# Hfx-J/SGTD

Measured on AMD Instinct MI355X. Metric: query frames/sec vs map size (descriptor build + candidate selection), higher is better.
Workload: dtype f64

## Files before the change

### sgtd_amd/csrc/order_kernels.hip.h

```cpp
#pragma once
#include "probe_kernels.hip.h"

#define SGTD_OS_THREADS 512
#define SGTD_OS_ITEMS 16
#define SGTD_OS_TILE (SGTD_OS_THREADS * SGTD_OS_ITEMS)
#define SGTD_GI_THREADS 256
#define SGTD_GI_ITEMS 16
#define SGTD_GI_TILE (SGTD_GI_THREADS * SGTD_GI_ITEMS)
#define SGTD_ORDER_WINDOW 8
#define SGTD_ORDER_POLLS_DEFAULT (1u << 20)
#define SGTD_ORDER_MAX_KEYS (1ll << 30)

enum { OW_TICKET = 0, OW_GROUP_TICKET = 4, OW_HIST = 64, OW_STATE = OW_HIST + 4 * 256 };
__host__ __device__ __forceinline__ size_t order_sort_state_at(int pass, u32 tiles_cap) { return (size_t)OW_STATE + (size_t)pass * tiles_cap * 256; }
__host__ __device__ __forceinline__ size_t order_group_state_at(int passes, u32 tiles_cap) { return (order_sort_state_at(passes, tiles_cap) + 1) & ~(size_t)1; }
__host__ __device__ __forceinline__ size_t order_work_words(int passes, u32 tiles_cap, u32 gtiles_cap) { return order_group_state_at(passes, tiles_cap) + (size_t)gtiles_cap * 2; }

#define SGTD_ST_AGG 1u
#define SGTD_ST_INCL 2u
#define SGTD_ST_MASK 0x3FFFFFFFu

__device__ __forceinline__ u32 order_ld(const u32 *p) { return __hip_atomic_load(p, __ATOMIC_RELAXED, __HIP_MEMORY_SCOPE_AGENT); }
__device__ __forceinline__ void order_st(u32 *p, u32 v) { __hip_atomic_store(p, v, __ATOMIC_RELAXED, __HIP_MEMORY_SCOPE_AGENT); }
__device__ __forceinline__ u64 order_ld64(const u64 *p) { return __hip_atomic_load(p, __ATOMIC_RELAXED, __HIP_MEMORY_SCOPE_AGENT); }
__device__ __forceinline__ void order_st64(u64 *p, u64 v) { __hip_atomic_store(p, v, __ATOMIC_RELAXED, __HIP_MEMORY_SCOPE_AGENT); }

__global__ __launch_bounds__(256) void order_begin_kernel(const u32 *count, u32 *q_prefix, int n_queries, u32 *n_valid, u32 *q_M, unsigned long long *q_P) {
  __shared__ u32 lds[256 / SGTD_WAVE + 1];
  for (int q = threadIdx.x; q < n_queries; q += 256) { q_M[q] = 0u; q_P[q] = 0ull; }
  u32 carry = 0;
  for (int q0 = 0; q0 < n_queries; q0 += 256) {
    const int q = q0 + threadIdx.x;
    const u32 v = (q < n_queries) ? count[q] : 0;
    u32 tot;
    const u32 ex = block_excl_scan(v, lds, tot);
    if (q < n_queries) q_prefix[q] = carry + ex;
    carry += tot;
  }
  if (threadIdx.x == 0) *n_valid = carry;
}

__global__ __launch_bounds__(256) void home_keys_hist_kernel(QueryView Q, const u32 *q_prefix, u32 *keys, u32 *vals, long long n_slots, int cbits, int sub_bits,
                                                             u32 *hist, u32 *pos_of_slot, size_t n_pass_slots) {
  __shared__ u32 h[4 * 256];
  for (int i = threadIdx.x; i < 4 * 256; i += 256) h[i] = 0u;
  __syncthreads();
  const u64 cmask = (1ull << cbits) - 1ull;
  const int ny = 1 << (sub_bits >> 1), nz = 1 << (sub_bits - (sub_bits >> 1));
  for (long long d = (long long)blockIdx.x * 256 + threadIdx.x; d < n_slots; d += (long long)gridDim.x * 256) {
    const int q = (int)(d / Q.stride);
    const u32 i = (u32)(d - (long long)q * Q.stride);
    if (i >= Q.count[q]) continue;
    const u64 code = label_code(Q.label[d * 3 + 0], Q.label[d * 3 + 1], Q.label[d * 3 + 2]);
    const double s0 = Q.side[d * 3 + 0], s1 = Q.side[d * 3 + 1], s2 = Q.side[d * 3 + 2];
    const u64 x = home_coord(s0, cmask), y = home_coord(s1, cmask), z = home_coord(s2, cmask);
    const double f1 = s1 - (double)(int)s1, f2 = s2 - (double)(int)s2;
    const u64 sub = (u64)min(max((int)(f1 * ny), 0), ny - 1) * nz + (u64)min(max((int)(f2 * nz), 0), nz - 1);
    const u32 key = (u32)(((((code << cbits | x) << cbits | y) << cbits) | z) << sub_bits | sub);
    const u32 idx = q_prefix[q] + i;
    keys[idx] = key;
    vals[idx] = (u32)d;
#pragma unroll
    for (int b = 0; b < 4; b++) atomicAdd(&h[b * 256 + ((key >> (8 * b)) & 255u)], 1u);
  }
  __syncthreads();
  for (int i = threadIdx.x; i < 4 * 256; i += 256)
    if (h[i]) atomicAdd(&hist[i], h[i]);
  uint4 *p4 = reinterpret_cast<uint4 *>(pos_of_slot);
  const size_t n4 = n_pass_slots / 4, step = (size_t)gridDim.x * 256, first = (size_t)blockIdx.x * 256 + threadIdx.x;
  for (size_t i = first; i < n4; i += step) p4[i] = make_uint4(SGTD_NO_PASS, SGTD_NO_PASS, SGTD_NO_PASS, SGTD_NO_PASS);
  for (size_t i = n4 * 4 + first; i < n_pass_slots; i += step) pos_of_slot[i] = SGTD_NO_PASS;
}

__global__ __launch_bounds__(SGTD_OS_THREADS) __attribute__((amdgpu_waves_per_eu(4))) void order_sort_pass_kernel(
const u32 *keys_in, const u32 *vals_in, u32 *keys_out, u32 *vals_out,
                                                                          const u32 *n_valid_p, long long n_cap, u32 *work, u32 tiles_cap, int pass,
                                                                          u32 max_polls, u32 *giveup) {
  constexpr int NW = SGTD_OS_THREADS / SGTD_WAVE;
  constexpr u32 PER_WAVE = SGTD_OS_TILE / NW;
  __shared__ u32 s_key[SGTD_OS_TILE], s_val[SGTD_OS_TILE];
  __shared__ u32 s_wcnt[NW][256];
  __shared__ u32 s_start[256];
  __shared__ u32 s_gbase[256];
  __shared__ u32 s_scan[NW + 1];
  __shared__ u32 s_tile, s_quit;
  const u32 tid = threadIdx.x, wid = tid >> 6, lane = tid & 63u;
  const u32 nv = (u32)min((long long)*n_valid_p, n_cap);
  const u32 ntiles = min((nv + SGTD_OS_TILE - 1u) / SGTD_OS_TILE, tiles_cap);
  if (blockIdx.x >= ntiles) return;
  if (tid == 0) { s_tile = atomicAdd(&work[OW_TICKET + pass], 1u); s_quit = order_ld(giveup); }
  for (u32 i = tid; i < NW * 256u; i += SGTD_OS_THREADS) (&s_wcnt[0][0])[i] = 0u;
  __syncthreads();
  const u32 tile = s_tile;
  if (s_quit || tile >= ntiles) return;
// ... 189 lines not shown
    s_heads = c_heads; s_last = c_last;
  }
  __syncthreads();
  if (s_quit) return;
  u32 H = s_heads + ex_heads, F = ex_last ? ex_last : s_last;
  u32 g[SGTD_GI_ITEMS];
#pragma unroll
  for (int j = 0; j < SGTD_GI_ITEMS; j++) {
    const u32 p = p0 + j;
    if ((heads >> j) & 1u) { H++; F = p + 1u; }
    g[j] = H - 1u;
    if (p < nv) {
      if (((heads >> j) & 1u) && H <= nv) group_first[H - 1u] = p;
      if (!pair) pos_of_slot[p] = p;
      else {
        const u32 f = F - 1u;
        if (((p - f) % SGTD_PAIR) == 0u) {
          const u32 s = (H - 1u) + (f + SGTD_PAIR - 1u) / SGTD_PAIR + (p - f) / SGTD_PAIR;
          if (s < slot_cap) pos_of_slot[s] = p;
        }
      }
      if (p == nv - 1u) *n_groups = H;
    }
  }
  if (full) {
    uint4 *dst = reinterpret_cast<uint4 *>(gid + p0);
#pragma unroll
    for (int j = 0; j < SGTD_GI_ITEMS / 4; j++) dst[j] = make_uint4(g[4 * j], g[4 * j + 1], g[4 * j + 2], g[4 * j + 3]);
  } else {
#pragma unroll
    for (int j = 0; j < SGTD_GI_ITEMS; j++) if (p0 + j < nv) gid[p0 + j] = g[j];
  }
}
```

### sgtd_amd/csrc/probe_kernels.hip.h

```cpp
#pragma once
#include "common.hip.h"
#include <type_traits>

struct TableView {
  const HotEntry *ent;
  IdMap map;
  const double *cold_side;
  const BucketDir *dir;
  const HashSlot *hash;
  u32 hash_mask;
  u32 n_entries;
  u32 frame_lo;
  u32 frame_span;
  u32 coarse_at;
  u32 whole_at;
  u32 tail_off;
  const BucketDir *dir1;
  const HashSlot *hash1;
  u32 hash_mask1;
  u32 n_entries1;
};
__host__ __device__ __forceinline__ u32 group_row_bytes(const TableView &T) { return T.tail_off ? 2u * SGTD_GROUP_ROW_BYTES : SGTD_GROUP_ROW_BYTES; }

struct QueryView {
// ... 64 lines not shown
struct WaveSlab {
  u32 state;
  u64 swept;
#ifdef SGTD_EXP_PHASE
  u64 ph[8], t;
#endif
};
#ifdef SGTD_EXP_PHASE
__device__ unsigned long long g_phase[8];
#define PH_ADD(i) do { const u64 _n = __builtin_readcyclecounter(); slab.ph[i] += _n - slab.t; slab.t = _n; } while (0)
#else
#define PH_ADD(i) do { } while (0)
#endif

__global__ __launch_bounds__(256) void query_prefix_kernel(const u32 *count, u32 *q_prefix, int n_queries,
                                                           u32 *n_valid) {
  __shared__ u32 lds[256 / SGTD_WAVE + 1];
  u32 carry = 0;
  for (int q0 = 0; q0 < n_queries; q0 += 256) {
    const int q = q0 + threadIdx.x;
    const u32 v = (q < n_queries) ? count[q] : 0;
    u32 tot;
    const u32 ex = block_excl_scan(v, lds, tot);
    if (q < n_queries) q_prefix[q] = carry + ex;
    carry += tot;
  }
  if (threadIdx.x == 0) *n_valid = carry;
}

__device__ __forceinline__ u64 home_coord(double s, u64 cmask) {
  return (int)(s - 1.0) < 0 ? cmask : min((u64)(u32)(int)s, cmask);
}

template <class KeyT>
__global__ void home_keys_kernel(QueryView Q, const u32 *q_prefix, KeyT *keys, u32 *vals, long long n_slots,
                                 int cbits, int sub_bits) {
  const long long d = (long long)blockIdx.x * blockDim.x + threadIdx.x;
  if (d >= n_slots) return;
  const int q = (int)(d / Q.stride);
  const u32 i = (u32)(d - (long long)q * Q.stride);
  if (i >= Q.count[q]) return;
  const u64 code = label_code(Q.label[d * 3 + 0], Q.label[d * 3 + 1], Q.label[d * 3 + 2]);
  const u64 cmask = (1ull << cbits) - 1ull;
  const u64 x = home_coord(Q.side[d * 3 + 0], cmask), y = home_coord(Q.side[d * 3 + 1], cmask),
            z = home_coord(Q.side[d * 3 + 2], cmask);
  const u32 idx = q_prefix[q] + i;
  const int ny = 1 << (sub_bits >> 1), nz = 1 << (sub_bits - (sub_bits >> 1));
  const double f1 = Q.side[d * 3 + 1] - (double)(int)Q.side[d * 3 + 1], f2 = Q.side[d * 3 + 2] - (double)(int)Q.side[d * 3 + 2];
  const u64 sub = (u64)min(max((int)(f1 * ny), 0), ny - 1) * nz + (u64)min(max((int)(f2 * nz), 0), nz - 1);
  keys[idx] = (KeyT)(((((code << cbits | x) << cbits | y) << cbits) | z) << sub_bits | sub);
  vals[idx] = (u32)d;
}

template <class KeyT>
__global__ void group_heads_kernel(const KeyT *keys, const u32 *n_valid_p, u32 *flags, long long n, int cbits, int sub_bits) {
  const long long p = (long long)blockIdx.x * blockDim.x + threadIdx.x;
  if (p >= n) return;
  u32 head = 0;
  if (p + 1 < (long long)*n_valid_p) {
    const u64 a = (u64)keys[p + 1] >> sub_bits, b = (u64)keys[p] >> sub_bits;
    const u64 cmask = (1ull << cbits) - 1ull;
    head = (a != b) || ((a & cmask) == cmask) || (((a >> cbits) & cmask) == cmask) ||
           (((a >> (2 * cbits)) & cmask) == cmask);
  }
  flags[p] = head;
}

__global__ void group_first_kernel(const u32 *gid, const u32 *n_valid_p, u32 *group_first, u32 *n_groups, long long n) {
  const long long p = (long long)blockIdx.x * blockDim.x + threadIdx.x;
  const long long nv = (long long)*n_valid_p;
  if (p >= n || p >= nv) return;
  const u32 g = gid[p];
  if (p == 0 || gid[p - 1] != g) group_first[g] = (u32)p;
  if (p == nv - 1) *n_groups = g + 1;
}

__global__ __launch_bounds__(256) void group_resolve_kernel(TableView T, QueryView Q, const u32 *order,
                                                            const u32 *group_first, const u32 *n_groups_p,
                                                            const u32 *n_valid_p, unsigned char *rows, u32 rows_cap,
                                                            int *overflow) {
  const int c = (int)(threadIdx.x & 31);
  const long long stride = ((long long)gridDim.x * blockDim.x) >> 5;
  const long long n_groups = (*n_valid_p) ? (long long)*n_groups_p : 0;
  if (n_groups > (long long)rows_cap) {
// ... 180 lines not shown
      head = (a != b) || ((a & cmask) == cmask) || (((a >> S.cbits) & cmask) == cmask) || (((a >> (2 * S.cbits)) & cmask) == cmask);
    }
    fl[j] = head;
    mine += head;
  }
  u32 tot;
  u32 ex = block_excl_scan(mine, s_sum, tot);
#pragma unroll
  for (u32 j = 0; j < PER; j++) {
    const u32 p = tid * PER + j;
    s_gid[p] = ex;
    if (p < S.n_slots) { S.gid[p] = ex; if (p < nv) S.order[p] = (u32)(s_key[p] & 8191ull); }
    ex += fl[j];
  }
  __syncthreads();
  for (u32 p = tid; p < nv; p += SGTD_SMALL_THREADS) {
    const u32 g = s_gid[p];
    if (p == 0 || s_gid[p - 1] != g) { s_first[g] = p; S.group_first[g] = p; }
  }
  if (tid == 0) { *S.n_valid = nv; *S.n_groups = nv ? s_gid[nv - 1] + 1u : 0u; }
  __syncthreads();
  for (u32 p = tid; p < nv; p += SGTD_SMALL_THREADS) {
    if (!S.pair) { S.pos_of_slot[p] = p; continue; }
    const u32 g = s_gid[p], f = s_first[g];
    if (((p - f) % SGTD_PAIR) == 0u) S.pos_of_slot[g + (f + SGTD_PAIR - 1u) / SGTD_PAIR + (p - f) / SGTD_PAIR] = p;
  }
}

__device__ __forceinline__ void reached_slices(float dq, float t_up, int n, int &lo, int &hi) {
  const float a = ((dq - t_up) + 0.5f) * (float)n - 1e-4f;
  const float b = ((dq + t_up) + 0.5f) * (float)n + 1e-4f;
  lo = !(a > 0.0f) ? 0 : (a >= (float)n ? n : (int)a);
  hi = b < 0.0f ? -1 : (!(b < (float)n) ? n - 1 : (int)b);
}

#ifndef SGTD_PLAN_GROUPS
#define SGTD_PLAN_GROUPS 16
#endif
#define SGTD_PLAN_THREADS 256
#ifndef SGTD_PLAN_WAVES
#define SGTD_PLAN_WAVES __attribute__((amdgpu_waves_per_eu(5)))
#endif
#ifndef SGTD_PLAN_INFLIGHT
#define SGTD_PLAN_INFLIGHT 4u
#endif
#ifndef SGTD_PLAN_SPARSE
#define SGTD_PLAN_SPARSE 1
#endif
#ifndef SGTD_PLAN_QUADS
#define SGTD_PLAN_QUADS 448
#endif
#define SGTD_ROW_QUADS (2 * SGTD_NCELL + 1)
template <bool PAIR, bool TAIL>
__global__ __launch_bounds__(SGTD_PLAN_THREADS) SGTD_PLAN_WAVES void plan_passes_kernel(TableView T, QueryView Q, const u32 *order, const u32 *gid,
                                                          const u32 *pos_of_slot, const u32 *n_valid_p,
                                                          const u32 *n_groups_p, const unsigned char *rows, u32 rows_cap, PassPool P,
                                                          u32 *n_visit, uint2 *list, int *overflow) {
  constexpr u32 SEGS = TAIL ? 2u : 1u;
  constexpr u32 NG = SGTD_PLAN_GROUPS / SEGS;
  constexpr size_t ROWB = (size_t)SEGS * SGTD_GROUP_ROW_BYTES;
  __shared__ uint4 s_rows[SGTD_PLAN_THREADS / SGTD_WAVE][SGTD_PLAN_QUADS + 2];
  const int lane = lane_id();
  uint4 *my_rows = s_rows[threadIdx.x >> 6];
  if (lane < 2) my_rows[lane] = make_uint4(0u, 0u, 0u, 0u);
  __builtin_amdgcn_wave_barrier();
  const u32 nv = *n_valid_p;
// ... 1400 lines not shown
```

### sgtd_amd/csrc/sgtd_accel.hip

```cpp
#include "../../include/sgtd_accel.h"

#include <hip/hip_runtime.h>

#include <algorithm>
#include <atomic>
#include <chrono>
#include <cmath>
#include <cstdio>
#include <cstring>
#include <limits>
#include <memory>
#include <string>
#include <vector>

#include "build_kernel.hip.h"
#include "common.hip.h"
#include "table_kernels.hip.h"
#include "probe_kernels.hip.h"
#include "order_kernels.hip.h"
#include "select_kernels.hip.h"
#include "verify_kernels.hip.h"
#include "verify_mfma.hip.h"
#include "exchange_kernels.hip.h"
#include "remove_kernels.hip.h"
// ... 60 lines not shown
  T *p = nullptr;
  size_t n = 0, cap = 0;
  PinnedVec() = default;
  PinnedVec(const PinnedVec &) = delete;
  PinnedVec &operator=(const PinnedVec &) = delete;
  ~PinnedVec() { if (p) (void)hipHostFree(p); }
  bool resize(size_t want) {
    if (want > cap) {
      void *np = nullptr;
      const size_t c = std::max<size_t>(want + want / 4, 64);
      if (hipHostMalloc(&np, c * sizeof(T), hipHostMallocDefault) != hipSuccess) return false;
      if (p) (void)hipHostFree(p);
      p = static_cast<T *>(np);
      cap = c;
    }
    n = want;
    return true;
  }
  T *data() { return p; }
  const T *data() const { return p; }
  T &operator[](size_t i) { return p[i]; }
  const T &operator[](size_t i) const { return p[i]; }
  size_t size() const { return n; }
};

constexpr size_t kCtrWords = CTR_XCD_HEADS + 8 * 1024;
enum { EV_START = 0, EV_BUILD, EV_SORT, EV_PROBE, EV_VOTES, EV_TOPK, EV_COUNT_T, EV_SCAN, EV_WRITE, EV_COUNT };

struct SelectPlan {
  int nq = 0, cn = 0; long long n_slots = 0; u32 span = 1, frame_lo = 0, id_bits = 13;
  u32 chunk = SGTD_PROBE_CHUNK; int blocks = 0, groups = 0, agrid = 0;
  u32 tile_span = 1, n_tiles = 1; size_t hist_bytes = 0; bool lds_votes = false;
  bool votes_fit = false, table_fits = false, per_query = false, fused_pairs = false, fused_votes = false, votes_per_query = false;
  int cbits = 1, sub_bits = 0, key_bits = 0; bool small = false, pair = false; size_t max_pass_slots = 0;
  bool order_fused = false; u32 order_tiles = 0, order_gtiles = 0;
  int row_slots = 1; u32 ticket = 2; int sgrid = 0, pgrid = 0; bool narrow = false, frames = false;
  bool narrow_pairs = false;
};

}

namespace multi { struct Group; }

struct sgtd_engine {
  multi::Group *grp = nullptr;
  sgtd_config cfg;
  DevCfg dc;
  hipStream_t stream = nullptr;
  std::string err;
  int n_cus = 256;
  bool timing = false;
  hipEvent_t ev[EV_COUNT] = {};

  sgtd_engine *attached_to = nullptr;
  unsigned long long table_version = 0;
  unsigned long long attached_version = 0;
  int n_views = 0;
  u32 current_frame_id = 0;
  DescStore tab;
  int64_t n_entries = 0;
  int64_t n_add_calls = 0;
  bool have_frames = false;
  u32 frame_lo = 0, frame_hi = 0;
  bool finalized = false;

  struct Segment {
// ... 128 lines not shown
  std::vector<int64_t> sk_off, sk_kp_off;
  enum { LM_POSE = 0, LM_OFF, LM_ANCH, LM_COUNT, LM_MERGED, LM_MEM_OFF, LM_MEMBER, LM_SEG, LM_CNT, LM_START, LM_MPTS, LM_MLAB, LM_XYZ, LM_LABEL,
         LM_NPOINTS, LM_BUFS };
  DevBuf lm[LM_BUFS];
  int lm_n = -1, lm_passes = 0;
  int64_t lm_kept = 0;
  std::vector<int64_t> lm_kp_off, lm_mem_off, lm_merged;
  hipEvent_t lm_ev[3] = {nullptr, nullptr, nullptr};
  float lm_ms[3] = {0.f, 0.f, 0.f};
  int *export_packed = nullptr;
  size_t export_cap = 0;
  hipEvent_t ev_cand = nullptr, ev_export_free = nullptr;
  bool export_busy = false;
  u32 batch_serial = 0;
  bool defer_lists = false;
  bool lists_pending = false;
  bool lists_masked = false;
  const u64 *verify_keep = nullptr;
  const u64 *list_keep = nullptr;
  SelectPlan plan;
  DevBuf rough_qi, rough_entry, rough_frame, rough_cell, rough_dis;
  size_t rec_cap = (size_t)1 << 25;
  bool rec_cap_fixed = false;
  size_t pair_cap = (size_t)1 << 24;
  DevBuf n_valid, cell_rows, gid, q_prefix, group_first, n_groups;
  DevBuf pos_of_slot, rec_off, pass_pool;
  size_t pool_units = 0;
  size_t group_cap = 0;
  size_t group_cap_hook = 0;
  size_t amb_min = 65536;
  int sorted_chunk = 0;
  bool diag = false;
  int order_form = -1;
  u32 order_polls = SGTD_ORDER_POLLS_DEFAULT;
  bool order_gave_up = false;
  bool order_train = false;
  int select_mode = 0;
  PinnedVec<u32> h_count, h_pair_base, h_q_M;
  PinnedVec<unsigned long long> h_q_P;
  PinnedVec<int> h_n_cand, h_cand_frame, h_cand_votes;
  PinnedVec<long long> h_pair_off;
  sgtd_stats stats{};
  char *pin = nullptr;
  size_t pin_cap = 0, pin_used = 0;
  struct PinCopy { void *dst; size_t off, bytes; };
  std::vector<PinCopy> pin_pending;
};

#include "multi.hip.h"

namespace {

#define HIPCHK(call)                                                          \
  do {                                                                        \
    hipError_t _s = (call);                                                   \
    if (_s != hipSuccess) {                                                   \
      e->err = std::string(#call) + ": " + hipGetErrorString(_s);             \
      return SGTD_ERR_HIP;                                                    \
    }                                                                         \
  } while (0)
#define CHK(call)                 \
  do {                            \
    int _r = (call);              \
    if (_r != SGTD_OK) return _r; \
  } while (0)

// ... 574 lines not shown
  SelectPlan p;
  const int nq = p.nq = e->nq, cn = p.cn = e->dc.cand_num;
  const long long n_slots = p.n_slots = (long long)nq * e->q_stride;
  const u32 span = p.span = e->have_frames ? (e->frame_hi - e->frame_lo + 1) : 1;
  p.frame_lo = e->have_frames ? e->frame_lo : 0;
  p.id_bits = e->id_bits ? e->id_bits : 13;
  while (p.chunk > SGTD_SUB_DESCS && (long long)nq * ((e->q_stride + p.chunk - 1) / p.chunk) < 1024) p.chunk >>= 1;
  if (const char *o = getenv("SGTD_BLOCK_CHUNK")) { const int c = atoi(o); if (c == 32 || c == 64 || c == 128) p.chunk = (u32)c; }
  p.blocks = (int)((e->q_stride + p.chunk - 1) / p.chunk);
  p.groups = (p.blocks + 3) / 4;
  p.agrid = ((nq + 7) / 8) * p.groups * 8;
  p.tile_span = span <= 36 * 1024 ? span : 36 * 1024;
  p.n_tiles = (span + p.tile_span - 1) / p.tile_span;
  p.hist_bytes = (size_t)span * sizeof(u32);
  p.lds_votes = p.hist_bytes <= 150 * 1024;
  static const size_t votes_room = lds_room(&votes_topk_kernel), list_room = lds_room(&pairs_query_kernel<true>);
  p.votes_fit = votes_topk_lds_bytes(span) <= votes_room;
  p.table_fits = (size_t)SGTD_PQ_TILE_RECS * sizeof(u32) + (((size_t)span + 15) & ~(size_t)15) + 16 <= list_room;
  p.per_query = e->select_mode == 2 || (e->select_mode == 0 && nq >= e->n_cus && (p.votes_fit || p.table_fits));
  p.fused_pairs = p.per_query && !e->wide_pairs && p.id_bits <= SGTD_PQ_RANK_BITS && !(cn == SGTD_MAX_CAND && p.id_bits == SGTD_PQ_RANK_BITS);
  p.fused_votes = p.fused_pairs && p.votes_fit;
  p.votes_per_query = p.n_tiles == 1 ? nq >= e->n_cus : ((long long)nq * p.n_tiles >= e->n_cus / 4 && p.n_tiles <= 8);
  p.narrow_pairs = p.id_bits <= SGTD_NARROW_RANK_BITS && !e->wide_pairs;
  while ((1ll << p.cbits) < (long long)(e->dc.max_len * e->dc.scale) + 3 && p.cbits < 16) p.cbits++;
  const int spare = (8 - (12 + 3 * p.cbits) % 8) % 8;
  p.sub_bits = spare >= 2 ? std::min(spare, 6) : 4;
  if (const char *o = getenv("SGTD_HOME_SUB_BITS")) p.sub_bits = std::min(6, std::max(0, atoi(o)));
  p.key_bits = 12 + 3 * p.cbits + p.sub_bits;
  const bool small_on = [] { const char *o = getenv("SGTD_SMALL_ORDER"); return !(o && !atoi(o)); }();
  p.small = small_on && nq == 1 && n_slots <= SGTD_SMALL_SLOTS && p.key_bits <= 32 && !p.fused_votes && span <= (1u << 20);
  const bool small_shape = nq == 1 && n_slots <= SGTD_SMALL_SLOTS;
  p.order_fused = !p.small && (e->order_form == 1 || (e->order_form < 0 && !small_shape)) && !e->order_train && p.key_bits <= 32 && n_slots > 0 &&
                  n_slots < SGTD_ORDER_MAX_KEYS;
  p.order_tiles = (u32)((n_slots + SGTD_OS_TILE - 1) / SGTD_OS_TILE);
  p.order_gtiles = (u32)((n_slots + SGTD_GI_TILE - 1) / SGTD_GI_TILE);
  p.pair = !e->diag && SGTD_PAIR >= 2;
  p.max_pass_slots = (size_t)pass_slot_count((u32)n_slots, (u32)n_slots, p.pair) + 64;
  p.row_slots = e->n_seg > 1 ? 2 : 1;
  if (e->stats.last_D > 0 && e->stats.last_P_swept > 0) {
    const double per_pass = (double)e->stats.last_P_swept / ((double)e->stats.last_D / (p.pair ? kDescsPerPass : 1.0));
    p.ticket = (u32)std::min(8.0, std::max(1.0, std::floor(1536.0 / per_pass + 0.5)));
  }
  if (e->sorted_chunk > 0) p.ticket = (u32)std::min(SGTD_TICKET_MAX, e->sorted_chunk);
  p.sgrid = e->n_cus * 8;
  if (const char *o = getenv("SGTD_SWEEP_BLOCKS_PER_CU")) p.sgrid = e->n_cus * std::max(1, atoi(o));
  int plan_per_cu = 20;
  if (const char *o = getenv("SGTD_PLAN_BLOCKS_PER_CU")) plan_per_cu = std::max(1, atoi(o));
  p.pgrid = (int)std::min<long long>(grid_for((long long)p.max_pass_slots, SGTD_PLAN_THREADS), (long long)e->n_cus * plan_per_cu);
  const u32 n0 = (u32)(e->seg[0].g1 - e->seg[0].g0), n1 = (u32)(e->seg[1].g1 - e->seg[1].g0);
  p.narrow = ((unsigned long long)n0 + SGTD_SENTINELS + (e->n_seg > 1 ? n1 + SGTD_SENTINELS : 0u)) * sizeof(HotEntry) < (1ull << 32);
  p.frames = e->last_kind != 1 || (e->have_frames && e->last_qframe >= e->frame_lo && e->last_qframe <= e->frame_hi);
  return p;
}

Views make_views(sgtd_engine *e) {
  const SelectPlan &p = e->plan;
  Views v;
  v.span = p.span;
  TableView &T = v.T;
  const sgtd_engine::Segment &S = e->seg[0], &S1 = e->seg[1];
  T.ent = S.hot.as<HotEntry>(); T.map = id_map(e, p.id_bits); T.cold_side = e->tab.side.as<double>();
  T.dir = S.dir.as<BucketDir>();
  T.hash = S.hash.as<HashSlot>(); T.hash_mask = S.hash_mask;
  T.coarse_at = e->coarse_at; T.whole_at = e->whole_at;
  T.n_entries = (u32)(S.g1 - S.g0); T.frame_lo = p.frame_lo; T.frame_span = v.span;
  T.tail_off = e->n_seg > 1 ? T.n_entries + SGTD_SENTINELS : 0u;
// ... 237 lines not shown
}

int clear_batch(sgtd_engine *e, const SelectPlan &p) {
  const int nq = p.nq, cn = p.cn;
  if (e->thr2_pending > 0) {
    thr2_kernel<<<grid_for(e->thr2_pending, 256), 256, 0, e->stream>>>(e->qd.side.as<double>(), e->qd.frame.as<u32>(), e->qd.qrec.as<QueryRec>(), e->thr2_pending,
                                                                        e->dc.rough);
    HIPCHK(hipGetLastError());
  }
  if (p.small) return SGTD_OK;
  HIPCHK(hipMemsetAsync(e->cursors.p, 0, kCtrWords * sizeof(u32), e->stream));
  if (!p.fused_votes) {
    if (!p.votes_per_query) HIPCHK(hipMemsetAsync(e->votes.p, 0, (size_t)nq * p.span * sizeof(u32), e->stream));
    HIPCHK(hipMemsetAsync(e->slot_of.p, 0xFF, (size_t)nq * p.span, e->stream));
    HIPCHK(hipMemsetAsync(e->cand_frame.p, 0xFF, (size_t)nq * cn * sizeof(int), e->stream));
    HIPCHK(hipMemsetAsync(e->cand_votes.p, 0, (size_t)nq * cn * sizeof(int), e->stream));
  }
  if (p.order_fused) return SGTD_OK;
  HIPCHK(hipMemsetAsync(e->q_M.p, 0, (size_t)nq * sizeof(u32), e->stream));
  HIPCHK(hipMemsetAsync(e->q_P.p, 0, (size_t)nq * sizeof(unsigned long long), e->stream));
  return SGTD_OK;
}

int order_fused(sgtd_engine *e, const SelectPlan &p, const Views &v, u32 **order) {
  const long long n_slots = p.n_slots;
  const int passes = (p.key_bits + 7) / 8;
  u32 *kin = e->keyA.as<u32>(), *kout = e->keyB.as<u32>(), *vin = e->valA.as<u32>(), *vout = e->valB.as<u32>();
  u32 *nv = e->n_valid.as<u32>(), *work = e->order_work.as<u32>(), *giveup = e->cursors.as<u32>() + CTR_ORDER_GIVEUP;
  order_begin_kernel<<<1, 256, 0, e->stream>>>(e->q_count.as<u32>(), e->q_prefix.as<u32>(), p.nq, nv, e->q_M.as<u32>(),
                                               e->q_P.as<unsigned long long>());
  HIPCHK(hipGetLastError());
  HIPCHK(hipMemsetAsync(work, 0, order_work_words(passes, p.order_tiles, p.order_gtiles) * sizeof(u32), e->stream));
  home_keys_hist_kernel<<<(unsigned)std::min<long long>(grid_for(n_slots, 256), (long long)e->n_cus * 8), 256, 0, e->stream>>>(v.Q, e->q_prefix.as<u32>(), kin, vin, n_slots,
                                                                                                                              p.cbits, p.sub_bits, work + OW_HIST, e->pos_of_slot.as<u32>(), p.max_pass_slots);
  HIPCHK(hipGetLastError());
  for (int pass = 0; pass < passes; pass++) {
    order_sort_pass_kernel<<<p.order_tiles, SGTD_OS_THREADS, 0, e->stream>>>(kin, vin, kout, vout, nv, n_slots, work, p.order_tiles, pass, e->order_polls, giveup);
    HIPCHK(hipGetLastError());
    std::swap(kin, kout);
    std::swap(vin, vout);
  }
  order_groups_kernel<<<p.order_gtiles, SGTD_GI_THREADS, 0, e->stream>>>(kin, nv, e->gid.as<u32>(), e->group_first.as<u32>(), e->n_groups.as<u32>(), e->pos_of_slot.as<u32>(),
                                                                        (u32)std::min<size_t>(p.max_pass_slots, 0xFFFFFFFFu), n_slots, work + OW_GROUP_TICKET,
                                                                        reinterpret_cast<u64 *>(work + order_group_state_at(passes, p.order_tiles)), p.order_gtiles, p.cbits,
                                                                        p.sub_bits, p.pair ? 1 : 0, e->order_polls, giveup, v.B.overflow());
  HIPCHK(hipGetLastError());
  e->thr2_pending = 0; *order = vin;
  return SGTD_OK;
}

int order_descriptors(sgtd_engine *e, const SelectPlan &p, const Views &v, u32 **order) {
  const long long n_slots = p.n_slots;
  u32 *vin = e->valA.as<u32>(), *vout = e->valB.as<u32>(), *gid = e->gid.as<u32>();
  const u32 *nv = e->n_valid.as<u32>();
  if (p.small) {
    SmallOrder SO;
    SO.ctr = e->cursors.as<u32>(); SO.ctr_words = (u32)kCtrWords;
    SO.q_M = e->q_M.as<u32>(); SO.q_P = e->q_P.as<unsigned long long>();
    SO.votes = p.votes_per_query ? nullptr : e->votes.as<u32>(); SO.slot_of_words = e->slot_of.as<u32>(); SO.span = p.span;
    SO.cand_frame = e->cand_frame.as<int>(); SO.cand_votes = e->cand_votes.as<int>(); SO.cand_num = p.cn;
    SO.q_prefix = e->q_prefix.as<u32>(); SO.n_valid = e->n_valid.as<u32>(); SO.order = vin; SO.gid = gid;
    SO.group_first = e->group_first.as<u32>(); SO.n_groups = e->n_groups.as<u32>(); SO.pos_of_slot = e->pos_of_slot.as<u32>();
    SO.n_slots = (u32)n_slots; SO.max_pass_slots = (u32)p.max_pass_slots; SO.cbits = p.cbits; SO.sub_bits = p.sub_bits; SO.pair = p.pair ? 1 : 0; SO.key_bits = p.key_bits;
    SO.qrec = nullptr; SO.n_qrec = 0; SO.rough = e->dc.rough;
    const size_t lds = (size_t)SGTD_SMALL_SLOTS * 16;
    HIPCHK(hipFuncSetAttribute(reinterpret_cast<const void *>(&small_order_kernel), hipFuncAttributeMaxDynamicSharedMemorySize, (int)lds));
    small_order_kernel<<<1, SGTD_SMALL_THREADS, lds, e->stream>>>(v.Q, SO);
    HIPCHK(hipGetLastError());
    e->thr2_pending = 0; *order = vin;
    return SGTD_OK;
  }
  if (p.order_fused) return order_fused(e, p, v, order);
  query_prefix_kernel<<<1, 256, 0, e->stream>>>(e->q_count.as<u32>(), e->q_prefix.as<u32>(), p.nq, e->n_valid.as<u32>());
  HIPCHK(hipGetLastError());
  auto sort_by_home = [&](auto *kin, auto *kout) -> int {
    using Key = typename std::remove_pointer<decltype(kin)>::type;
    home_keys_kernel<Key><<<grid_for(n_slots, 256), 256, 0, e->stream>>>(v.Q, e->q_prefix.as<u32>(), kin, vin, n_slots, p.cbits, p.sub_bits);
    HIPCHK(hipGetLastError());
    CHK(radix_sort_pairs(e, kin, kout, vin, vout, n_slots, p.key_bits, false, nv));
    group_heads_kernel<Key><<<grid_for(n_slots, 256), 256, 0, e->stream>>>(kin, nv, gid, n_slots, p.cbits, p.sub_bits);
    HIPCHK(hipGetLastError());
    return SGTD_OK;
  };
  if (p.key_bits <= 32) CHK(sort_by_home(e->keyA.as<u32>(), e->keyB.as<u32>()));
  else CHK(sort_by_home(e->keyA.as<u64>(), e->keyB.as<u64>()));
  CHK(device_scan(e, gid, gid, n_slots));
  group_first_kernel<<<grid_for(n_slots, 256), 256, 0, e->stream>>>(gid, nv, e->group_first.as<u32>(), e->n_groups.as<u32>(), n_slots);
  HIPCHK(hipGetLastError());
  HIPCHK(hipMemsetAsync(e->pos_of_slot.p, 0xFF, p.max_pass_slots * sizeof(u32), e->stream));
  pass_slots_kernel<<<grid_for(n_slots, 256), 256, 0, e->stream>>>(gid, e->group_first.as<u32>(), nv, e->pos_of_slot.as<u32>(), n_slots, p.pair ? 1 : 0);
  HIPCHK(hipGetLastError());
  e->thr2_pending = 0; *order = vin;
  return SGTD_OK;
}

int plan_and_sweep(sgtd_engine *e, const SelectPlan &p, const Views &v, u32 *vin) {
  const u32 *nv = e->n_valid.as<u32>();
  const unsigned char *rows = e->cell_rows.as<unsigned char>();
  const u32 rows_cap = (u32)std::min<size_t>(e->group_cap, 0xFFFFFFFFu);
  PassPool PP;
  PP.pool = e->pass_pool.as<uint4>(); PP.rec_off = e->rec_off.as<u32>();
  PP.cursor = v.B.pool_cursor(); PP.cap = (u32)std::min<size_t>(e->pool_units, 0xFFFFFF00u);
  group_resolve_kernel<<<e->n_cus * 16, 256, 0, e->stream>>>(v.T, v.Q, vin, e->group_first.as<u32>(),
                                                              e->n_groups.as<u32>(), nv, e->cell_rows.as<unsigned char>(), rows_cap, v.B.overflow());
  HIPCHK(hipGetLastError());
#define SGTD_LAUNCH_PLAN(PR, TL)                                                                               \
  plan_passes_kernel<PR, TL><<<p.pgrid, SGTD_PLAN_THREADS, 0, e->stream>>>(v.T, v.Q, vin, e->gid.as<u32>(), e->pos_of_slot.as<u32>(), nv, \
                                                       e->n_groups.as<u32>(), rows, rows_cap, PP, v.B.n_visit, v.B.list,          \
                                                       v.B.overflow())
  if (v.T.tail_off) { if (p.pair) SGTD_LAUNCH_PLAN(true, true); else SGTD_LAUNCH_PLAN(false, true); }
  else { if (p.pair) SGTD_LAUNCH_PLAN(true, false); else SGTD_LAUNCH_PLAN(false, false); }
#undef SGTD_LAUNCH_PLAN
  HIPCHK(hipGetLastError());
  if (e->timing) HIPCHK(hipEventRecord(e->ev[EV_SORT], e->stream));
#define SGTD_LAUNCH_SORTED(DG, WD, FR, BD)                                                                      \
  probe_sorted_kernel<DG, WD, FR, BD><<<p.sgrid, SGTD_PROBE_THREADS, 0, e->stream>>>(                           \
      v.T, v.B, v.Q, PP, e->dc.rough, e->n_valid.as<u32>(), e->n_groups.as<u32>(), p.ticket)
  if (e->diag) {
    if (e->loop_batch) SGTD_LAUNCH_SORTED(true, true, true, true);
    else SGTD_LAUNCH_SORTED(true, true, true, false);
  } else if (e->loop_batch) {
    if (p.narrow) SGTD_LAUNCH_SORTED(false, false, true, true);
    else SGTD_LAUNCH_SORTED(false, true, true, true);
  }
  else if (p.narrow && p.frames) SGTD_LAUNCH_SORTED(false, false, true, false);
// ... 79 lines not shown
  if (sl_bytes) CHK(p.narrow_pairs ? count(&block_count_kernel<true, true>) : count(&block_count_kernel<true, false>));
  else CHK(p.narrow_pairs ? count(&block_count_kernel<false, true>) : count(&block_count_kernel<false, false>));
  if (e->timing) HIPCHK(hipEventRecord(e->ev[EV_COUNT_T], e->stream));
  block_scan_kernel<<<nq, 64, 0, e->stream>>>(e->blk_count.as<u32>(), p.blocks, p.cn, e->n_cand.as<int>(),
                                               e->pair_off.as<long long>(), e->q_pairs.as<u32>(),
                                               v.B.overflow(), nq == 1 ? e->q_pair_base.as<u32>() : nullptr, pair_room(e),
                                               nq == 1 ? e->totals.as<unsigned long long>() : nullptr);
  HIPCHK(hipGetLastError());
  if (nq != 1) {
    query_base_kernel<<<1, 256, 0, e->stream>>>(e->q_pairs.as<u32>(), e->q_pair_base.as<u32>(), nq, pair_room(e), v.B.overflow());
    HIPCHK(hipGetLastError());
  }
  if (e->timing) HIPCHK(hipEventRecord(e->ev[EV_SCAN], e->stream));
  CHK(launch_block_write(e, p, v, CL));
  if (e->timing) HIPCHK(hipEventRecord(e->ev[EV_WRITE], e->stream));
  if (nq != 1) {
    batch_totals_kernel<<<1, 1, 0, e->stream>>>(v.B.ctr, e->totals.as<unsigned long long>());
    HIPCHK(hipGetLastError());
  }
  e->batch_valid = true;
  new_results(e, false);
  e->batch_synced = false;
  return SGTD_OK;
}

int launch_select(sgtd_engine *e) {
  e->plan = plan_select(e);
  const SelectPlan &p = e->plan;
  CHK(reserve_select(e, p));
  CHK(clear_batch(e, p));
  const Views v = make_views(e);
  u32 *order = nullptr;
  CHK(order_descriptors(e, p, v, &order));
  CHK(plan_and_sweep(e, p, v, order));
  CHK(launch_votes(e, p, v));
  CHK(launch_topk(e, p, v));
  CHK(export_candidates(e, v));
  e->lists_pending = false;
  e->lists_masked = false;
  e->stats.select_form = p.fused_votes ? 2 : (p.fused_pairs ? 1 : 0);
  if (!p.fused_pairs) return launch_block_lists(e, p, v);
  e->batch_valid = true;
  if (!e->defer_lists) return launch_lists(e, v, nullptr, true);
  if (e->timing)
    for (int k : {EV_COUNT_T, EV_SCAN, EV_WRITE}) HIPCHK(hipEventRecord(e->ev[k], e->stream));
  batch_totals_kernel<<<1, 1, 0, e->stream>>>(v.B.ctr, e->totals.as<unsigned long long>());
  HIPCHK(hipGetLastError());
  e->lists_pending = true;
  new_results(e, false);
  e->batch_synced = false;
  return SGTD_OK;
}

int enqueue_frames(sgtd_engine *e) {
  const int nq = e->nq;
  if (e->timing) HIPCHK(hipEventRecord(e->ev[EV_START], e->stream));
  CHK(launch_build(e, e->last_xyz, e->last_label, e->kp_off_dev.as<long long>(), nq, e->last_max_n,
                   e->last_qframe, e->loop_batch ? 1 : 0, e->qd.view(), e->q_stride, e->q_count.as<u32>()));
  if (e->loop_batch) {
    loop_bound_kernel<<<grid_for(e->q_stride * nq, 256), 256, 0, e->stream>>>(e->qd.qrec.as<QueryRec>(), e->q_stride, nq, e->last_qframe,
                                                                             e->loop_skip, e->have_frames ? e->frame_lo : 0);
    HIPCHK(hipGetLastError());
  }
  if (e->timing) HIPCHK(hipEventRecord(e->ev[EV_BUILD], e->stream));
  return launch_select(e);
}
// ... 346 lines not shown
uint64_t sgtd_table_key(uint32_t code, uint32_t x, uint32_t y, uint32_t z) { return pack_key(code, x, y, z); }
uint64_t sgtd_dedup_key(uint64_t mx, uint64_t my, uint64_t mz) { return pack_milli_key(mx, my, mz); }

int sgtd_create(const sgtd_config *cfg, sgtd_handle *out) {
  if (!cfg || !out) return SGTD_ERR_INVALID;
  *out = nullptr;
  int r = check_cfg(cfg);
  if (r != SGTD_OK) return r;
  int ndev = 0;
  if (hipGetDeviceCount(&ndev) != hipSuccess || ndev <= 0) return SGTD_ERR_NO_DEVICE;
  if (cfg->device_id < 0 || cfg->device_id >= ndev) return SGTD_ERR_NO_DEVICE;
  hipDeviceProp_t prop;
  if (hipGetDeviceProperties(&prop, cfg->device_id) != hipSuccess) return SGTD_ERR_NO_DEVICE;
  if (std::strncmp(prop.gcnArchName, "gfx950", 6) != 0) return SGTD_ERR_NO_DEVICE;
  if (hipSetDevice(cfg->device_id) != hipSuccess) return SGTD_ERR_NO_DEVICE;
  sgtd_engine *e = new sgtd_engine();
  e->cfg = *cfg;
  e->dc.K = cfg->descriptor_near_num;
  e->dc.tpi = (cfg->descriptor_near_num - 1) * (cfg->descriptor_near_num - 2) / 2;
  e->dc.cand_num = cfg->candidate_num;
  e->dc.min_len = cfg->descriptor_min_len;
  e->dc.max_len = cfg->descriptor_max_len;
  e->dc.scale = 1.0 / cfg->std_side_resolution;
  e->dc.rough = cfg->rough_dis_threshold;
  e->n_cus = prop.multiProcessorCount > 0 ? prop.multiProcessorCount : 256;
  e->current_frame_id = cfg->first_frame_id;
  e->qd.with_thr2 = true;
  if (const char *o = getenv("SGTD_SORTED_CHUNK")) e->sorted_chunk = atoi(o);
  if (const char *o = getenv("SGTD_TAIL_MAX")) e->tail_max = atoll(o);
  if (const char *o = getenv("SGTD_COARSE_AT")) e->coarse_at = (u32)std::min(62ll, std::max(0ll, atoll(o)));
  if (const char *o = getenv("SGTD_REC_RATE")) e->rec_rate_hook = (u32)std::min(256, std::max(1, atoi(o)));
  if (const char *o = getenv("SGTD_WIDE_PAIRS")) e->wide_pairs = atoi(o) != 0;
  if (const char *o = getenv("SGTD_ORDER_FORM")) e->order_form = atoi(o) != 0 ? 1 : 0;
  if (const char *o = getenv("SGTD_ORDER_POLLS")) e->order_polls = (u32)std::min(1ll << 30, std::max(0ll, atoll(o)));
  if (const char *o = getenv("SGTD_SELECT_MODE")) e->select_mode = std::min(2, std::max(0, atoi(o)));
  if (const char *o = getenv("SGTD_WHOLE_AT")) e->whole_at = (u32)std::min(62ll, std::max(0ll, atoll(o)));
  if (const char *o = getenv("SGTD_REC_CAP")) { e->rec_cap = (size_t)std::max(1024ll, atoll(o)); e->rec_cap_fixed = true; }
  if (const char *o = getenv("SGTD_POOL_UNITS")) e->pool_units = (size_t)std::max(64ll, atoll(o));
  if (const char *o = getenv("SGTD_GROUP_CAP")) e->group_cap_hook = (size_t)std::max(1ll, atoll(o));
  if (const char *o = getenv("SGTD_PAIR_CAP")) { e->pair_cap = (size_t)std::max(64ll, atoll(o)); e->rec_cap_fixed = true; }
  if (const char *o = getenv("SGTD_AMB_MIN")) e->amb_min = (size_t)std::max(1ll, atoll(o));
  for (int i = 0; i < EV_COUNT; i++)
    if (hipEventCreate(&e->ev[i]) != hipSuccess) { delete e; return SGTD_ERR_HIP; }
  if (hipEventCreateWithFlags(&e->ev_cand, hipEventDisableTiming) != hipSuccess ||
      hipEventCreateWithFlags(&e->ev_export_free, hipEventDisableTiming) != hipSuccess) { delete e; return SGTD_ERR_HIP; }
  *out = e;
  return SGTD_OK;
}

int sgtd_create_multi(const sgtd_config *cfg, const int *device_ids, int n_dev, sgtd_handle *out) {
  if (n_dev == 1 && cfg && device_ids && out) {
    sgtd_config c = *cfg;
    c.device_id = device_ids[0];
    return sgtd_create(&c, out);
  }
  return multi::create(cfg, device_ids, n_dev, out);
}

int sgtd_device_count(sgtd_handle e) { return !e ? 0 : (e->grp ? multi::device_count(e) : 1); }

sgtd_handle sgtd_device_handle(sgtd_handle e, int k) {
  if (!e) return nullptr;
  if (!e->grp) return k == 0 ? e : nullptr;
  return multi::device_handle(e, k);
}

// ... 3173 lines not shown
```

Before: 194,000.

## Reorder descriptors within home cells by reached-slice pattern tag

Computes an 8-bit tag per descriptor summarizing which y/z slices its search radius reaches and packs it into the upper bits of the sort value. A new kernel then re-sorts entries within each home-cell group inside a wavefront (bitonic sort on the tag) so neighboring lanes probe similar slice ranges. This is meant to reduce divergence and improve locality in the sweep, at the cost of an extra kernel, extra tag computation in key building, and a dependence on index bits fitting in 24 bits.

```diff
diff --git a/sgtd_amd/csrc/order_kernels.hip.h b/sgtd_amd/csrc/order_kernels.hip.h
--- a/sgtd_amd/csrc/order_kernels.hip.h
+++ b/sgtd_amd/csrc/order_kernels.hip.h
@@ -41,7 +41,7 @@
 }
 
 __global__ __launch_bounds__(256) void home_keys_hist_kernel(QueryView Q, const u32 *q_prefix, u32 *keys, u32 *vals, long long n_slots, int cbits, int sub_bits,
-                                                             u32 *hist, u32 *pos_of_slot, size_t n_pass_slots) {
+                                                             u32 *hist, u32 *pos_of_slot, size_t n_pass_slots, double rough, int tag_shift) {
   __shared__ u32 h[4 * 256];
   for (int i = threadIdx.x; i < 4 * 256; i += 256) h[i] = 0u;
   __syncthreads();
@@ -59,7 +59,7 @@
     const u32 key = (u32)(((((code << cbits | x) << cbits | y) << cbits) | z) << sub_bits | sub);
     const u32 idx = q_prefix[q] + i;
     keys[idx] = key;
-    vals[idx] = (u32)d;
+    vals[idx] = (u32)d | (tag_shift ? pass_tag(s0, s1, s2, rough) << tag_shift : 0u);
 #pragma unroll
     for (int b = 0; b < 4; b++) atomicAdd(&h[b * 256 + ((key >> (8 * b)) & 255u)], 1u);
   }
@@ -315,3 +315,34 @@
     for (int j = 0; j < SGTD_GI_ITEMS; j++) if (p0 + j < nv) gid[p0 + j] = g[j];
   }
 }
+
+__global__ __launch_bounds__(256) void order_refine_cells_kernel(const u32 *gid, u32 *order, const u32 *n_valid_p, long long n_cap, int tag_shift,
+                                                                 const u32 *giveup, const int *overflow) {
+  const u32 nv = (u32)min((long long)*n_valid_p, n_cap);
+  const int lane = (int)(threadIdx.x & 63u);
+  const long long p = (long long)blockIdx.x * 256 + threadIdx.x;
+  if (p - lane >= (long long)nv) return;
+  const bool valid = p < (long long)nv;
+  const u32 g = valid ? gid[p] : 0xFFFFFFFFu;
+  const u32 w = valid ? order[p] : 0u;
+  const u32 o = w & ((1u << tag_shift) - 1u), f = w >> tag_shift;
+  if (*giveup || overflow[0]) {
+    if (valid) order[p] = o;
+    return;
+  }
+  const u32 g_before = (u32)__shfl_up((int)g, 1);
+  const u64 heads = __builtin_amdgcn_ballot_w64(lane == 0 || g != g_before);
+  const u32 first = 63u - (u32)__builtin_clzll(heads & ((2ull << lane) - 1ull));
+  u32 key = first << 26 | min(f, 0xFFFFFu) << 6 | (u32)lane;
+#pragma unroll
+  for (int k = 2; k <= SGTD_WAVE; k <<= 1) {
+#pragma unroll
+    for (int j = k >> 1; j > 0; j >>= 1) {
+      const u32 other = (u32)__shfl_xor((int)key, j);
+      const bool low = ((lane & j) == 0) == ((lane & k) == 0 || k == SGTD_WAVE);
+      key = low ? min(key, other) : max(key, other);
+    }
+  }
+  const u32 from = (u32)__builtin_amdgcn_ds_bpermute((int)((key & 63u) << 2), (int)o);
+  if (valid) order[p] = from;
+}
diff --git a/sgtd_amd/csrc/probe_kernels.hip.h b/sgtd_amd/csrc/probe_kernels.hip.h
--- a/sgtd_amd/csrc/probe_kernels.hip.h
+++ b/sgtd_amd/csrc/probe_kernels.hip.h
@@ -120,9 +120,10 @@
   return (int)(s - 1.0) < 0 ? cmask : min((u64)(u32)(int)s, cmask);
 }
 
+__device__ __forceinline__ u32 pass_tag(double s0, double s1, double s2, double rough);
 template <class KeyT>
 __global__ void home_keys_kernel(QueryView Q, const u32 *q_prefix, KeyT *keys, u32 *vals, long long n_slots,
-                                 int cbits, int sub_bits) {
+                                 int cbits, int sub_bits, double rough, int tag_shift) {
   const long long d = (long long)blockIdx.x * blockDim.x + threadIdx.x;
   if (d >= n_slots) return;
   const int q = (int)(d / Q.stride);
@@ -137,7 +138,7 @@
   const double f1 = Q.side[d * 3 + 1] - (double)(int)Q.side[d * 3 + 1], f2 = Q.side[d * 3 + 2] - (double)(int)Q.side[d * 3 + 2];
   const u64 sub = (u64)min(max((int)(f1 * ny), 0), ny - 1) * nz + (u64)min(max((int)(f2 * nz), 0), nz - 1);
   keys[idx] = (KeyT)(((((code << cbits | x) << cbits | y) << cbits) | z) << sub_bits | sub);
-  vals[idx] = (u32)d;
+  vals[idx] = (u32)d | (tag_shift ? pass_tag(Q.side[d * 3 + 0], Q.side[d * 3 + 1], Q.side[d * 3 + 2], rough) << tag_shift : 0u);
 }
 
 template <class KeyT>
@@ -384,6 +385,26 @@
   const float b = ((dq + t_up) + 0.5f) * (float)n + 1e-4f;
   lo = !(a > 0.0f) ? 0 : (a >= (float)n ? n : (int)a);
   hi = b < 0.0f ? -1 : (!(b < (float)n) ? n - 1 : (int)b);
+}
+
+#define SGTD_PASS_TAG_BITS 8
+__device__ __forceinline__ u32 pass_tag(double s0, double s1, double s2, double rough) {
+  const double tm = norm3(s0, s1, s2) * rough * (1.0 + 1e-9) + 1e-12;
+  float t_up = (float)tm;
+  if ((double)t_up < tm) t_up = __uint_as_float(__float_as_uint(t_up) + 1u);
+  if (!(tm == tm)) t_up = __builtin_inff();
+  u32 ym = 0, zm = 0;
+#pragma unroll
+  for (int o = 0; o < 3; o++) {
+    int lo, hi;
+    reached_slices((float)(s1 - (double)(int)(s1 + (double)(o - 1))), t_up, SGTD_YSLICES, lo, hi);
+    ym |= (((1u << (hi + 1)) - 1u) & ~((1u << lo) - 1u)) << (2 * o);
+    reached_slices((float)(s2 - (double)(int)(s2 + (double)(o - 1))), t_up, SGTD_ZSLICES, lo, hi);
+    zm |= (((1u << (hi + 1)) - 1u) & ~((1u << lo) - 1u)) << (3 * o);
+  }
+  const u32 ys = ym ? (u32)__builtin_ctz(ym) : 6u, zs = zm ? (u32)__builtin_ctz(zm) : 9u;
+  const u32 ye = ym ? 31u - (u32)__builtin_clz(ym) : 6u, ze = zm ? 31u - (u32)__builtin_clz(zm) : 9u;
+  return (ys + ye) * 19u + (zs + ze);
 }
 
 #ifndef SGTD_PLAN_GROUPS
diff --git a/sgtd_amd/csrc/sgtd_accel.hip b/sgtd_amd/csrc/sgtd_accel.hip
--- a/sgtd_amd/csrc/sgtd_accel.hip
+++ b/sgtd_amd/csrc/sgtd_accel.hip
@@ -116,6 +116,7 @@
   u32 chunk = SGTD_PROBE_CHUNK; int blocks = 0, groups = 0, agrid = 0;
   u32 tile_span = 1, n_tiles = 1; size_t hist_bytes = 0; bool lds_votes = false;
   bool votes_fit = false, table_fits = false, per_query = false, fused_pairs = false, fused_votes = false, votes_per_query = false;
+  int tag_shift = 0;
   int cbits = 1, sub_bits = 0, key_bits = 0; bool small = false, pair = false; size_t max_pass_slots = 0;
   bool order_fused = false; u32 order_tiles = 0, order_gtiles = 0;
   int row_slots = 1; u32 ticket = 2; int sgrid = 0, pgrid = 0; bool narrow = false, frames = false;
@@ -310,6 +311,7 @@
   int sorted_chunk = 0;
   bool diag = false;
   int order_form = -1;
+  bool pass_order = true;
   u32 order_polls = SGTD_ORDER_POLLS_DEFAULT;
   bool order_gave_up = false;
   bool order_train = false;
@@ -950,6 +952,12 @@
   const bool small_shape = nq == 1 && n_slots <= SGTD_SMALL_SLOTS;
   p.order_fused = !p.small && (e->order_form == 1 || (e->order_form < 0 && !small_shape)) && !e->order_train && p.key_bits <= 32 && n_slots > 0 &&
                   n_slots < SGTD_ORDER_MAX_KEYS;
+  p.tag_shift = 0;
+  if (e->pass_order && !p.small && n_slots > 0) {
+    int bits = 1;
+    while ((1ll << bits) < n_slots) bits++;
+    if (bits + SGTD_PASS_TAG_BITS <= 32) p.tag_shift = bits;
+  }
   p.order_tiles = (u32)((n_slots + SGTD_OS_TILE - 1) / SGTD_OS_TILE);
   p.order_gtiles = (u32)((n_slots + SGTD_GI_TILE - 1) / SGTD_GI_TILE);
   p.pair = !e->diag && SGTD_PAIR >= 2;
@@ -1253,7 +1261,8 @@
   HIPCHK(hipGetLastError());
   HIPCHK(hipMemsetAsync(work, 0, order_work_words(passes, p.order_tiles, p.order_gtiles) * sizeof(u32), e->stream));
   home_keys_hist_kernel<<<(unsigned)std::min<long long>(grid_for(n_slots, 256), (long long)e->n_cus * 8), 256, 0, e->stream>>>(v.Q, e->q_prefix.as<u32>(), kin, vin, n_slots,
-                                                                                                                              p.cbits, p.sub_bits, work + OW_HIST, e->pos_of_slot.as<u32>(), p.max_pass_slots);
+                                                                                                                              p.cbits, p.sub_bits, work + OW_HIST, e->pos_of_slot.as<u32>(), p.max_pass_slots,
+                                                                                                                              e->dc.rough, p.tag_shift);
   HIPCHK(hipGetLastError());
   for (int pass = 0; pass < passes; pass++) {
     order_sort_pass_kernel<<<p.order_tiles, SGTD_OS_THREADS, 0, e->stream>>>(kin, vin, kout, vout, nv, n_slots, work, p.order_tiles, pass, e->order_polls, giveup);
@@ -1296,7 +1305,7 @@
   HIPCHK(hipGetLastError());
   auto sort_by_home = [&](auto *kin, auto *kout) -> int {
     using Key = typename std::remove_pointer<decltype(kin)>::type;
-    home_keys_kernel<Key><<<grid_for(n_slots, 256), 256, 0, e->stream>>>(v.Q, e->q_prefix.as<u32>(), kin, vin, n_slots, p.cbits, p.sub_bits);
+    home_keys_kernel<Key><<<grid_for(n_slots, 256), 256, 0, e->stream>>>(v.Q, e->q_prefix.as<u32>(), kin, vin, n_slots, p.cbits, p.sub_bits, e->dc.rough, p.tag_shift);
     HIPCHK(hipGetLastError());
     CHK(radix_sort_pairs(e, kin, kout, vin, vout, n_slots, p.key_bits, false, nv));
     group_heads_kernel<Key><<<grid_for(n_slots, 256), 256, 0, e->stream>>>(kin, nv, gid, n_slots, p.cbits, p.sub_bits);
@@ -1312,6 +1321,14 @@
   pass_slots_kernel<<<grid_for(n_slots, 256), 256, 0, e->stream>>>(gid, e->group_first.as<u32>(), nv, e->pos_of_slot.as<u32>(), n_slots, p.pair ? 1 : 0);
   HIPCHK(hipGetLastError());
   e->thr2_pending = 0; *order = vin;
+  return SGTD_OK;
+}
+
+int refine_order(sgtd_engine *e, const SelectPlan &p, const Views &v, u32 *order) {
+  if (!p.tag_shift) return SGTD_OK;
+  order_refine_cells_kernel<<<grid_for(p.n_slots, 256), 256, 0, e->stream>>>(e->gid.as<u32>(), order, e->n_valid.as<u32>(), p.n_slots, p.tag_shift,
+                                                                             e->cursors.as<u32>() + CTR_ORDER_GIVEUP, v.B.overflow());
+  HIPCHK(hipGetLastError());
   return SGTD_OK;
 }
 
@@ -1457,6 +1474,7 @@
   const Views v = make_views(e);
   u32 *order = nullptr;
   CHK(order_descriptors(e, p, v, &order));
+  CHK(refine_order(e, p, v, order));
   CHK(plan_and_sweep(e, p, v, order));
   CHK(launch_votes(e, p, v));
   CHK(launch_topk(e, p, v));
@@ -1869,6 +1887,7 @@
   if (const char *o = getenv("SGTD_REC_RATE")) e->rec_rate_hook = (u32)std::min(256, std::max(1, atoi(o)));
   if (const char *o = getenv("SGTD_WIDE_PAIRS")) e->wide_pairs = atoi(o) != 0;
   if (const char *o = getenv("SGTD_ORDER_FORM")) e->order_form = atoi(o) != 0 ? 1 : 0;
+  if (const char *o = getenv("SGTD_PASS_ORDER")) e->pass_order = atoi(o) != 0;
   if (const char *o = getenv("SGTD_ORDER_POLLS")) e->order_polls = (u32)std::min(1ll << 30, std::max(0ll, atoll(o)));
   if (const char *o = getenv("SGTD_SELECT_MODE")) e->select_mode = std::min(2, std::max(0, atoi(o)));
   if (const char *o = getenv("SGTD_WHOLE_AT")) e->whole_at = (u32)std::min(62ll, std::max(0ll, atoll(o)));
```

Result: no change. 192,500 (-0.8%).
